# afermg/aliby

Hardware: AMD Instinct MI355X
Metric: FOV tiles/sec (whole node) (higher is better)
Workload: dtype u16 pixels, f64 feature accumulators, f32 dynamics, bfloat16 U-Net

## Files before the change

aliby_amd/csrc/feat_coloc.hip:

```cpp
#include "common.h"
#include "object_launch.h"
#include "coloc_stats.h"

typedef unsigned short u16;

struct ColocArgs {
  const u16* labels;
  const void* planes;
  int F, C, Y, X, ch0, ch1;
  const aliby_object* tab;
  int n_obj;
  int cap;
  unsigned char* gscratch;
  double* out;
  int ld;
  int col_pearson, col_manders, col_rwc, col_costes;
  double thr;
  double scale_max;
  const unsigned int* ranks;
  const int* rmax;
};

struct PlaneRanks {
  const unsigned int* rk1;
  const unsigned int* rk2;
  const int* rmax;
  int ch0, ch1;
  __device__ __forceinline__ double R() const { return (double)(max(rmax[ch0], rmax[ch1]) + 1); }
  __device__ __forceinline__ long long diff(int j) const { return llabs((long long)rk1[j] - (long long)rk2[j]); }
};

template <typename T, bool GLOBAL>
__global__ __launch_bounds__(256) void k_coloc(ColocArgs a) {
  extern __shared__ __align__(16) unsigned char lds_raw[];
  __shared__ double vec[4 * 8];
  __shared__ double red_d[8];
  __shared__ float red_f[8];
  __shared__ int red_i[8];
  __shared__ int wsum[4];
  unsigned char* ws = GLOBAL ? (a.gscratch + (size_t)blockIdx.x * (size_t)a.cap * 16) : lds_raw;
  float* fv = reinterpret_cast<float*>(ws);
  float* sv = fv + a.cap;
  unsigned int* rk1 = reinterpret_cast<unsigned int*>(sv + a.cap);
  unsigned int* rk2 = rk1 + a.cap;
  const int tid = threadIdx.x;
  const size_t plane = (size_t)a.Y * a.X;

  for (int oi = blockIdx.x; oi < a.n_obj; oi += gridDim.x) {
    const aliby_object o = a.tab[oi];
    double* out = a.out + (size_t)oi * a.ld;
    if (o.area <= 0) {
      if (tid == 0) {
        if (a.col_pearson >= 0) { out[a.col_pearson] = NAN; out[a.col_pearson + 1] = NAN; }
        if (a.col_manders >= 0) { out[a.col_manders] = NAN; out[a.col_manders + 1] = NAN; }
        if (a.col_rwc >= 0) { out[a.col_rwc] = NAN; out[a.col_rwc + 1] = NAN; }
        if (a.col_costes >= 0) { out[a.col_costes] = NAN; out[a.col_costes + 1] = NAN; }
      }
      continue;
    }
    const u16* lab = a.labels + (size_t)o.tile * plane;
    const T* p0 = reinterpret_cast<const T*>(a.planes) + ((size_t)o.tile * a.C + a.ch0) * plane;
    const T* p1 = reinterpret_cast<const T*>(a.planes) + ((size_t)o.tile * a.C + a.ch1) * plane;
    const int h = o.y1 - o.y0, w = o.x1 - o.x0, npix = h * w;
    const u16 L = (u16)o.label;

    __syncthreads();
    int base = 0;
    for (int i0 = 0; i0 < npix; i0 += blockDim.x) {
      const int i = i0 + tid;
      bool in = false;
      size_t idx = 0;
      if (i < npix) {
        idx = (size_t)(o.y0 + i / w) * a.X + (o.x0 + i % w);
        in = lab[idx] == L;
      }
      const int pos = block_compact_slot(in, base, wsum);
      if (in) {
        fv[pos] = px_load<T>(p0, idx); sv[pos] = px_load<T>(p1, idx);
        if (a.col_rwc >= 0) {
          rk1[pos] = a.ranks[((size_t)o.tile * a.C + a.ch0) * plane + idx];
          rk2[pos] = a.ranks[((size_t)o.tile * a.C + a.ch1) * plane + idx];
        }
      }
    }
    __syncthreads();
    const int N = base;
    coloc_block_stats(fv, sv, N, out, a.col_pearson, a.col_manders, a.col_rwc, a.col_costes, a.thr, a.scale_max,
                      PlaneRanks{rk1, rk2, a.rmax + (size_t)oi * a.C, a.ch0, a.ch1}, vec, red_f, red_i);
    (void)red_d;
    __syncthreads();
  }
}


#define COLOC_MAX_CH 8
#define COLOC_MAX_PAIRS 28
struct PairsArgs {
  const u16* labels;
  const void* planes;
  int F, C, Y, X;
  const aliby_object* tab;
  int n_obj, cap;
  double* out;
  int ld;
  double thr, scale_max;
  const unsigned int* ranks;
  const int* rmax;
  int nch, npairs, any_rwc;
  int chan[COLOC_MAX_CH];
  int pair[COLOC_MAX_PAIRS][6];
};

template <int K>
__device__ __forceinline__ void wave_sum_all(double (&v)[K]) {
#pragma unroll
  for (int k = 0; k < K; ++k) v[k] = wave_sum(v[k]);
}

template <typename T>
__global__ __launch_bounds__(256) void k_coloc_pairs(PairsArgs a) {
  extern __shared__ __align__(16) unsigned char lds_raw[];
  __shared__ int wsum[4];
  float* vals = reinterpret_cast<float*>(lds_raw);
  unsigned int* rks = reinterpret_cast<unsigned int*>(vals + (size_t)a.nch * a.cap);
  const int tid = threadIdx.x, lane = tid & 63, wave = tid >> 6;
  const size_t plane = (size_t)a.Y * a.X;

  for (int oi = blockIdx.x; oi < a.n_obj; oi += gridDim.x) {
    const aliby_object o = a.tab[oi];
    double* out = a.out + (size_t)oi * a.ld;
    if (o.area <= 0) {
      for (int p = tid; p < a.npairs; p += blockDim.x)
        for (int k = 2; k < 6; ++k)
          if (a.pair[p][k] >= 0) { out[a.pair[p][k]] = NAN; out[a.pair[p][k] + 1] = NAN; }
      continue;
    }
    const u16* lab = a.labels + (size_t)o.tile * plane;
    const T* img = reinterpret_cast<const T*>(a.planes) + (size_t)o.tile * a.C * plane;
    const int h = o.y1 - o.y0, w = o.x1 - o.x0, npix = h * w;
    const u16 L = (u16)o.label;
    __syncthreads();
    int base = 0;
    for (int i0 = 0; i0 < npix; i0 += blockDim.x) {
      const int i = i0 + tid;
      bool in = false;
      size_t idx = 0;
      if (i < npix) {
        idx = (size_t)(o.y0 + i / w) * a.X + (o.x0 + i % w);
        in = lab[idx] == L;
      }
      const int pos = block_compact_slot(in, base, wsum);
      if (in) {
        for (int c = 0; c < a.nch; ++c) {
          vals[(size_t)c * a.cap + pos] = px_load<T>(img + (size_t)a.chan[c] * plane, idx);
          if (a.any_rwc) rks[(size_t)c * a.cap + pos] = a.ranks[((size_t)o.tile * a.C + a.chan[c]) * plane + idx];
        }
      }
    }
    __syncthreads();
    const int N = base;
    const double dN = (double)N;

    for (int p = wave; p < a.npairs; p += 4) {
      const int ca = a.pair[p][0], cb = a.pair[p][1];
      const int col_pearson = a.pair[p][2], col_manders = a.pair[p][3], col_rwc = a.pair[p][4], col_costes = a.pair[p][5];
      const float* fv = vals + (size_t)ca * a.cap;
      const float* sv = vals + (size_t)cb * a.cap;
      const unsigned int* rk1 = rks + (size_t)ca * a.cap;
      const unsigned int* rk2 = rks + (size_t)cb * a.cap;

      double s2[2] = {0, 0};
      float m1 = -INFINITY, m2 = -INFINITY;
      for (int j = lane; j < N; j += 64) {
        s2[0] += (double)fv[j]; s2[1] += (double)sv[j];
        m1 = fmaxf(m1, fv[j]); m2 = fmaxf(m2, sv[j]);
      }
      wave_sum_all<2>(s2);
      const double mean1 = s2[0] / dN, mean2 = s2[1] / dN;
      const float MAX1 = wave_max(m1), MAX2 = wave_max(m2);

      if (col_pearson >= 0) {
        double q[3] = {0, 0, 0};
        for (int j = lane; j < N; j += 64) {
          const double x = (double)fv[j] - mean1, y = (double)sv[j] - mean2;
          q[0] += x * x; q[1] += y * y; q[2] += x * y;
        }
        wave_sum_all<3>(q);
        if (lane == 0) {
          out[col_pearson] = q[2] / (sqrt(q[0]) * sqrt(q[1]));
          out[col_pearson + 1] = q[2] / q[0];
        }
      }

      const double tff = (a.thr / 100.0) * (double)MAX1, tss = (a.thr / 100.0) * (double)MAX2;
      double tot1 = 0, tot2 = 0;
      int any_comb = 0;
      if (col_manders >= 0 || col_rwc >= 0) {
        double q[4] = {0, 0, 0, 0};
        int anyc = 0;
        for (int j = lane; j < N; j += 64) {
          const double f = fv[j], s = sv[j];
          const bool a1 = f >= tff, a2 = s >= tss;
          if (a1) q[0] += f;
          if (a2) q[1] += s;
          if (a1 && a2) { q[2] += f; q[3] += s; anyc = 1; }
        }
        wave_sum_all<4>(q);
        any_comb = wave_max(anyc);
        tot1 = q[0]; tot2 = q[1];
        if (col_manders >= 0 && lane == 0) {
          out[col_manders] = any_comb ? q[2] / tot1 : 0.0;
          out[col_manders + 1] = any_comb ? q[3] / tot2 : 0.0;
        }
      }

      if (col_rwc >= 0) {
        const double R = (double)(max(a.rmax[(size_t)oi * a.C + a.chan[ca]], a.rmax[(size_t)oi * a.C + a.chan[cb]]) + 1);
        double q[2] = {0, 0};
        for (int j = lane; j < N; j += 64) {
          const double f = fv[j], s = sv[j];
          if (f >= tff && s >= tss) {
            const long long di = llabs((long long)rk1[j] - (long long)rk2[j]);
            const double wgt = (R - (double)di) * 1.0 / R;
            q[0] += f * wgt; q[1] += s * wgt;
          }
        }
        wave_sum_all<2>(q);
        if (lane == 0) {
          out[col_rwc] = any_comb ? q[0] / tot1 : 0.0;
          out[col_rwc + 1] = any_comb ? q[1] / tot2 : 0.0;
        }
      }

      if (col_costes >= 0) {
        double q[3] = {0, 0, 0};
        for (int j = lane; j < N; j += 64) {
          const double f = fv[j], s = sv[j];
          if (f > 0 || s > 0) { q[0] += 1; q[1] += f; q[2] += s; }
        }
        wave_sum_all<3>(q);
        const double nnz = q[0], xmean = q[1] / nnz, ymean = q[2] / nnz, zmean = (q[1] + q[2]) / nnz;
        double v3[3] = {0, 0, 0};
        for (int j = lane; j < N; j += 64) {
          const double f = fv[j], s = sv[j];
          if (f > 0 || s > 0) {
            const double dx = f - xmean, dy = s - ymean, dz = (f + s) - zmean;
            v3[0] += dx * dx; v3[1] += dy * dy; v3[2] += dz * dz;
          }
        }
        wave_sum_all<3>(v3);
        const double xvar = v3[0] / (nnz - 1), yvar = v3[1] / (nnz - 1), zvar = v3[2] / (nnz - 1);
        const double covar = 0.5 * (zvar - (xvar + yvar));
        const double denom = 2 * covar;
        const double num = (yvar - xvar) + sqrt((yvar - xvar) * (yvar - xvar) + 4 * (covar * covar));
        const double cA = num / denom, cB = ymean - cA * xmean;
        double left = 1, right = a.scale_max;
      const bool int_bounds = a.scale_max == floor(a.scale_max) && a.scale_max >= 1 && a.scale_max <= 1048576.0;
        double mid = floor((right - left) / (6.0 / 5.0)) + left;
        double lastmid = 0, valid = 1;
        for (int it = 0; it < 200 && lastmid != mid; ++it) {
          const double t1 = mid / a.scale_max, t2 = cA * t1 + cB;
          double c3[3] = {0, 0, 0};
          for (int j = lane; j < N; j += 64) {
            const double f = fv[j], s = sv[j];
            if (f < t1 || s < t2) { c3[0] += 1; c3[1] += f; c3[2] += s; }
          }
          wave_sum_all<3>(c3);
          if (c3[0] <= 2) {
            left = mid - 1;
          } else {
            const double mx = c3[1] / c3[0], my = c3[2] / c3[0];
            double p3[3] = {0, 0, 0};
            for (int j = lane; j < N; j += 64) {
              const double f = fv[j], s = sv[j];
              if (f < t1 || s < t2) { const double dx = f - mx, dy = s - my; p3[0] += dx * dx; p3[1] += dy * dy; p3[2] += dx * dy; }
            }
            wave_sum_all<3>(p3);
            if (p3[0] != 0 && p3[1] != 0) {
              if (p3[2] < 0) left = mid - 1;
              else if (p3[2] >= 0) { right = mid + 1; valid = mid; }
            }
          }
          lastmid = mid;
          mid = costes_next_mid(left, right, int_bounds);
        }
        const double t1 = (valid - 1) / a.scale_max, t2 = cA * t1 + cB;
        double c4[4] = {0, 0, 0, 0};
        int f_any = 0, s_any = 0, c_any = 0;
        for (int j = lane; j < N; j += 64) {
          const double f = fv[j], s = sv[j];
          const bool fa = f > t1, sa = s > t2;
          f_any |= fa; s_any |= sa;
          if (f >= t1) c4[0] += f;
          if (s >= t2) c4[1] += s;
          if (fa && sa) { c4[2] += f; c4[3] += s; c_any = 1; }
        }
        wave_sum_all<4>(c4);
        const int FA = wave_max(f_any), SA = wave_max(s_any), CA = wave_max(c_any);
        if (lane == 0) {
          const double d1 = FA ? c4[0] : 0.0, d2 = SA ? c4[1] : 0.0;
          out[col_costes] = CA ? c4[2] / d1 : 0.0;
          out[col_costes + 1] = CA ? c4[3] / d2 : 0.0;
        }
      }
    }
  }
}


struct RankArgs {
  const u16* labels;
  const void* planes;
  int F, C, Y, X, channel;
  const aliby_object* tab;
  int n_obj, cap;
  unsigned char* gscratch;
  unsigned int* ranks;
  int* rmax;
};

template <typename T, bool GLOBAL>
__global__ __launch_bounds__(256) void k_ranks(RankArgs a) {
  extern __shared__ __align__(16) unsigned char lds_raw[];
  __shared__ int wsum[4];
  __shared__ int part[256];
  unsigned char* ws = GLOBAL ? (a.gscratch + (size_t)blockIdx.x * (size_t)a.cap * 16) : lds_raw;
  float* vals = reinterpret_cast<float*>(ws);
  float* S = vals + a.cap;
  int* P = reinterpret_cast<int*>(S + a.cap);
  int* pix = P + a.cap;
  const int tid = threadIdx.x;
  const size_t plane = (size_t)a.Y * a.X;
  for (int oi = blockIdx.x; oi < a.n_obj; oi += gridDim.x) {
    const aliby_object o = a.tab[oi];
    if (o.area <= 0) { if (tid == 0) a.rmax[(size_t)oi * a.C + a.channel] = 0; continue; }
    const u16* lab = a.labels + (size_t)o.tile * plane;
    const T* px = reinterpret_cast<const T*>(a.planes) + ((size_t)o.tile * a.C + a.channel) * plane;
    unsigned int* rk = a.ranks + ((size_t)o.tile * a.C + a.channel) * plane;
    const int h = o.y1 - o.y0, w = o.x1 - o.x0, npix = h * w;
    const u16 L = (u16)o.label;
    __syncthreads();
    int base = 0;
    for (int i0 = 0; i0 < npix; i0 += blockDim.x) {
      const int i = i0 + tid;
      bool in = false;
      size_t idx = 0;
      if (i < npix) { idx = (size_t)(o.y0 + i / w) * a.X + (o.x0 + i % w); in = lab[idx] == L; }
      const int pos = block_compact_slot(in, base, wsum);
      if (in) { vals[pos] = px_load<T>(px, idx); pix[pos] = (int)idx; }
    }
    __syncthreads();
    const int N = base;
    bool done = false;
    if (sizeof(T) == 2 && !GLOBAL) {
      int lo = INT_MAX, hi = 0;
      for (int j = tid; j < N; j += blockDim.x) { const int v = (int)vals[j]; lo = min(lo, v); hi = max(hi, v); }
      const int vmin = block_min_i32(lo, part), vmax = block_max_i32(hi, part);
      const int w0 = vmin >> 5, nw = (vmax >> 5) - w0 + 1;
      if (nw <= a.cap) {
        unsigned int* bits = reinterpret_cast<unsigned int*>(S);
        __syncthreads();
        for (int i = tid; i < nw; i += blockDim.x) bits[i] = 0u;
        __syncthreads();
        for (int j = tid; j < N; j += blockDim.x) { const int v = (int)vals[j]; atomicOr(&bits[(v >> 5) - w0], 1u << (v & 31)); }
        __syncthreads();
        for (int i = tid; i < nw; i += blockDim.x) P[i] = __popc(bits[i]);
        __syncthreads();
        block_inclusive_scan(P, nw, part);
        for (int j = tid; j < N; j += blockDim.x) {
          const int v = (int)vals[j], wi = (v >> 5) - w0;
          const unsigned int below = bits[wi] & ((1u << (v & 31)) - 1u);
          rk[pix[j]] = (unsigned int)(P[wi] - __popc(bits[wi]) + __popc(below));
        }
        if (tid == 0) a.rmax[(size_t)oi * a.C + a.channel] = P[nw - 1] - 1;
        done = true;
      }
    }
    if (done) { __syncthreads(); continue; }
    const int n2 = next_pow2(N);
    for (int i = tid; i < n2; i += blockDim.x) S[i] = (i < N) ? vals[i] : INFINITY;
    block_bitonic_sort(S, n2);
    for (int i = tid; i < N; i += blockDim.x) P[i] = (i > 0 && S[i] != S[i - 1]) ? 1 : 0;
    __syncthreads();
    block_inclusive_scan(P, N, part);
    for (int j = tid; j < N; j += blockDim.x) {
      const float v = vals[j];
      int lo = 0, hi = N;
      while (lo < hi) { const int mid = (lo + hi) >> 1; if (S[mid] < v) lo = mid + 1; else hi = mid; }
      rk[pix[j]] = (unsigned int)P[lo];
    }
    if (tid == 0) a.rmax[(size_t)oi * a.C + a.channel] = P[N - 1];
    __syncthreads();
  }
}

extern "C" int aliby_object_ranks(aliby_ctx* ctx, const uint16_t* labels, const void* planes, int dtype, int F, int C,
                                  int Y, int X, int channel, const aliby_object* table_dev, int n_obj, int max_area,
                                  uint32_t* ranks_dev, int32_t* rmax_dev, void* stream) {
  ARG_CHECK(ctx != nullptr, "ctx is NULL");
  if (n_obj == 0) return ALIBY_OK;
  ARG_CHECK(labels && planes && table_dev && ranks_dev && rmax_dev, "NULL argument");
  ARG_CHECK(dtype == ALIBY_U16 || dtype == ALIBY_F32, "dtype must be ALIBY_U16 or ALIBY_F32");
  ARG_CHECK(channel >= 0 && channel < C, "channel out of range");
  ARG_CHECK((size_t)Y * X < (size_t)INT_MAX, "plane too large");
  RankArgs a;
  a.labels = labels; a.planes = planes; a.F = F; a.C = C; a.Y = Y; a.X = X; a.channel = channel; a.tab = table_dev;
  a.n_obj = n_obj; a.ranks = ranks_dev; a.rmax = rmax_dev;
  a.cap = aliby_pow2_at_least(max_area, 64);
  return object_launch(ctx, object_kernel(dtype, k_ranks<u16, false>, k_ranks<float, false>),
                       object_kernel(dtype, k_ranks<u16, true>, k_ranks<float, true>), a, n_obj, (size_t)a.cap * 16, 96 * 1024, max_area,
                       as_stream(stream));
}

extern "C" int aliby_features_coloc(aliby_ctx* ctx, const uint16_t* labels, const void* planes, int dtype,
                                    int F, int C, int Y, int X, int ch0, int ch1,
                                    const aliby_object* table_dev, int n_obj, int max_area,
                                    double* out, int ld, int col_pearson, int col_manders, int col_rwc,
                                    int col_costes, double thr_percent, double costes_scale_max,
                                    const uint32_t* ranks_dev, const int32_t* rmax_dev, void* stream) {
  ARG_CHECK(ctx != nullptr, "ctx is NULL");
  if (n_obj == 0) return ALIBY_OK;
  ARG_CHECK(labels && planes && table_dev && out, "NULL argument");
  ARG_CHECK(dtype == ALIBY_U16 || dtype == ALIBY_F32, "dtype must be ALIBY_U16 or ALIBY_F32");
  ARG_CHECK(ch0 >= 0 && ch0 < C && ch1 >= 0 && ch1 < C, "channel out of range");
  ARG_CHECK(F > 0 && Y > 0 && X > 0 && max_area >= 0, "bad shape");
  const int cols[4] = {col_pearson, col_manders, col_rwc, col_costes};
  for (int k = 0; k < 4; ++k) ARG_CHECK(cols[k] < 0 || cols[k] + 2 <= ld, "columns exceed row stride");
  ColocArgs a;
  a.labels = labels; a.planes = planes; a.F = F; a.C = C; a.Y = Y; a.X = X; a.ch0 = ch0; a.ch1 = ch1;
  a.tab = table_dev; a.n_obj = n_obj; a.out = out; a.ld = ld;
  a.col_pearson = col_pearson; a.col_manders = col_manders; a.col_rwc = col_rwc; a.col_costes = col_costes;
  a.thr = thr_percent; a.scale_max = costes_scale_max;
  a.ranks = ranks_dev; a.rmax = rmax_dev;
  ARG_CHECK(col_rwc < 0 || (ranks_dev && rmax_dev), "rwc needs the rank planes (aliby_object_ranks)");
  a.cap = aliby_pow2_at_least(max_area, 64);
  return object_launch(ctx, object_kernel(dtype, k_coloc<u16, false>, k_coloc<float, false>),
                       object_kernel(dtype, k_coloc<u16, true>, k_coloc<float, true>), a, n_obj, (size_t)a.cap * 16, 96 * 1024, max_area,
                       as_stream(stream));
}

extern "C" int aliby_features_coloc_pairs(aliby_ctx* ctx, const uint16_t* labels, const void* planes, int dtype, int F, int C,
                                          int Y, int X, const int32_t* pairs_host, int n_pairs,
                                          const aliby_object* table_dev, int n_obj, int max_area, double* out, int ld,
                                          double thr_percent, double costes_scale_max, const uint32_t* ranks_dev,
                                          const int32_t* rmax_dev, void* stream) {
  ARG_CHECK(ctx != nullptr, "ctx is NULL");
  if (n_obj == 0 || n_pairs == 0) return ALIBY_OK;
  ARG_CHECK(labels && planes && table_dev && out && pairs_host, "NULL argument");
  ARG_CHECK(dtype == ALIBY_U16 || dtype == ALIBY_F32, "dtype must be ALIBY_U16 or ALIBY_F32");
  ARG_CHECK(F > 0 && Y > 0 && X > 0 && max_area >= 0, "bad shape");
  ARG_CHECK(n_pairs > 0 && n_pairs <= COLOC_MAX_PAIRS, "too many channel pairs for one launch");
  PairsArgs a;
  a.labels = labels; a.planes = planes; a.F = F; a.C = C; a.Y = Y; a.X = X; a.tab = table_dev; a.n_obj = n_obj;
  a.out = out; a.ld = ld; a.thr = thr_percent; a.scale_max = costes_scale_max; a.ranks = ranks_dev; a.rmax = rmax_dev;
  a.nch = 0; a.npairs = n_pairs; a.any_rwc = 0;
  for (int p = 0; p < n_pairs; ++p) {
    const int32_t* q = pairs_host + 6 * p;
    for (int k = 0; k < 2; ++k) {
      ARG_CHECK(q[k] >= 0 && q[k] < C, "channel out of range");
      int loc = -1;
      for (int c = 0; c < a.nch; ++c) if (a.chan[c] == q[k]) loc = c;
      if (loc < 0) {
        ARG_CHECK(a.nch < COLOC_MAX_CH, "too many distinct channels for one launch");
        loc = a.nch;
        a.chan[a.nch++] = q[k];
      }
      a.pair[p][k] = loc;
    }
    for (int k = 2; k < 6; ++k) {
      ARG_CHECK(q[k] < 0 || q[k] + 2 <= ld, "columns exceed row stride");
      a.pair[p][k] = q[k];
    }
    if (q[4] >= 0) a.any_rwc = 1;
  }
  ARG_CHECK(!a.any_rwc || (ranks_dev && rmax_dev), "rwc needs the rank planes (aliby_object_ranks)");
  a.cap = aliby_pow2_at_least(max_area, 64);
  const size_t need = (size_t)a.nch * a.cap * 4 * (a.any_rwc ? 2 : 1);
  if (need > 144 * 1024) {
    aliby_set_error("coloc_pairs: %zu bytes of pixel lists per object exceed the LDS budget", need);
    return ALIBY_ERR_TOO_LARGE;
  }
  hipStream_t s = as_stream(stream);
  auto k = object_kernel(dtype, k_coloc_pairs<u16>, k_coloc_pairs<float>);
  HIP_TRY(hipFuncSetAttribute((const void*)k, hipFuncAttributeMaxDynamicSharedMemorySize, 144 * 1024));
  hipLaunchKernelGGL(k, dim3(n_obj), dim3(256), need, s, a);
  KERNEL_CHECK();
  return ALIBY_OK;
}
```

Measured before the change: 604.4.

## Shrink LDS pixel and rank lists to u16 and window the rank bitset

The coloc pairs kernel now stores u16 pixel values and u16 ranks in LDS instead of float/uint32, sizes lists to a multiple of 64 rather than a power of two, and skips the shared-memory attribute call when it is not needed. For u16 inputs, the rank kernel gets a dedicated path that keeps u16 values and 16-bit positions in LDS. It builds the dense-rank bitset in fixed 256-word windows in static LDS, so the sort fallback is no longer used. The aim is to cut LDS footprint so more blocks fit per CU, and to avoid the bitonic sort. The cost is extra per-window passes when the value range is wide, plus a rescan path for very large objects.

```diff
diff --git a/aliby_amd/csrc/feat_coloc.hip b/aliby_amd/csrc/feat_coloc.hip
--- a/aliby_amd/csrc/feat_coloc.hip
+++ b/aliby_amd/csrc/feat_coloc.hip
@@ -95,6 +95,7 @@
 
 #define COLOC_MAX_CH 8
 #define COLOC_MAX_PAIRS 28
+#define COLOC_PAIRS_LDS_BUDGET (144 * 1024)
 struct PairsArgs {
   const u16* labels;
   const void* planes;
@@ -117,12 +118,24 @@
   for (int k = 0; k < K; ++k) v[k] = wave_sum(v[k]);
 }
 
+template <typename T> struct PairRank { typedef unsigned int type; };
+template <> struct PairRank<u16> { typedef u16 type; };
+static_assert((1u << (8 * sizeof(u16))) - 1u <= (PairRank<u16>::type)~0u, "the largest dense rank of uint16 pixels must fit the rank lists");
+
+static inline int list_cap64(int max_area) { return max_area <= 64 ? 64 : (max_area + 63) / 64 * 64; }
+static inline size_t coloc_pairs_need(int dtype, int nch, int cap, int any_rwc) {
+  const size_t v = dtype == ALIBY_U16 ? sizeof(u16) : sizeof(float);
+  const size_t r = dtype == ALIBY_U16 ? sizeof(PairRank<u16>::type) : sizeof(PairRank<float>::type);
+  return (size_t)nch * cap * (v + (any_rwc ? r : 0));
+}
+
 template <typename T>
 __global__ __launch_bounds__(256) void k_coloc_pairs(PairsArgs a) {
+  typedef typename PairRank<T>::type R;
   extern __shared__ __align__(16) unsigned char lds_raw[];
   __shared__ int wsum[4];
-  float* vals = reinterpret_cast<float*>(lds_raw);
-  unsigned int* rks = reinterpret_cast<unsigned int*>(vals + (size_t)a.nch * a.cap);
+  T* vals = reinterpret_cast<T*>(lds_raw);
+  R* rks = reinterpret_cast<R*>(vals + (size_t)a.nch * a.cap);
   const int tid = threadIdx.x, lane = tid & 63, wave = tid >> 6;
   const size_t plane = (size_t)a.Y * a.X;
 
@@ -152,8 +165,8 @@
       const int pos = block_compact_slot(in, base, wsum);
       if (in) {
         for (int c = 0; c < a.nch; ++c) {
-          vals[(size_t)c * a.cap + pos] = px_load<T>(img + (size_t)a.chan[c] * plane, idx);
-          if (a.any_rwc) rks[(size_t)c * a.cap + pos] = a.ranks[((size_t)o.tile * a.C + a.chan[c]) * plane + idx];
+          vals[(size_t)c * a.cap + pos] = img[(size_t)a.chan[c] * plane + idx];
+          if (a.any_rwc) rks[(size_t)c * a.cap + pos] = (R)a.ranks[((size_t)o.tile * a.C + a.chan[c]) * plane + idx];
         }
       }
     }
@@ -164,16 +177,16 @@
     for (int p = wave; p < a.npairs; p += 4) {
       const int ca = a.pair[p][0], cb = a.pair[p][1];
       const int col_pearson = a.pair[p][2], col_manders = a.pair[p][3], col_rwc = a.pair[p][4], col_costes = a.pair[p][5];
-      const float* fv = vals + (size_t)ca * a.cap;
-      const float* sv = vals + (size_t)cb * a.cap;
-      const unsigned int* rk1 = rks + (size_t)ca * a.cap;
-      const unsigned int* rk2 = rks + (size_t)cb * a.cap;
+      const T* fv = vals + (size_t)ca * a.cap;
+      const T* sv = vals + (size_t)cb * a.cap;
+      const R* rk1 = rks + (size_t)ca * a.cap;
+      const R* rk2 = rks + (size_t)cb * a.cap;
 
       double s2[2] = {0, 0};
       float m1 = -INFINITY, m2 = -INFINITY;
       for (int j = lane; j < N; j += 64) {
-        s2[0] += (double)fv[j]; s2[1] += (double)sv[j];
-        m1 = fmaxf(m1, fv[j]); m2 = fmaxf(m2, sv[j]);
+        s2[0] += (double)(float)fv[j]; s2[1] += (double)(float)sv[j];
+        m1 = fmaxf(m1, (float)fv[j]); m2 = fmaxf(m2, (float)sv[j]);
       }
       wave_sum_all<2>(s2);
       const double mean1 = s2[0] / dN, mean2 = s2[1] / dN;
@@ -182,7 +195,7 @@
       if (col_pearson >= 0) {
         double q[3] = {0, 0, 0};
         for (int j = lane; j < N; j += 64) {
-          const double x = (double)fv[j] - mean1, y = (double)sv[j] - mean2;
+          const double x = (double)(float)fv[j] - mean1, y = (double)(float)sv[j] - mean2;
           q[0] += x * x; q[1] += y * y; q[2] += x * y;
         }
         wave_sum_all<3>(q);
@@ -199,7 +212,7 @@
         double q[4] = {0, 0, 0, 0};
         int anyc = 0;
         for (int j = lane; j < N; j += 64) {
-          const double f = fv[j], s = sv[j];
+          const double f = (float)fv[j], s = (float)sv[j];
           const bool a1 = f >= tff, a2 = s >= tss;
           if (a1) q[0] += f;
           if (a2) q[1] += s;
@@ -218,7 +231,7 @@
         const double R = (double)(max(a.rmax[(size_t)oi * a.C + a.chan[ca]], a.rmax[(size_t)oi * a.C + a.chan[cb]]) + 1);
         double q[2] = {0, 0};
         for (int j = lane; j < N; j += 64) {
-          const double f = fv[j], s = sv[j];
+          const double f = (float)fv[j], s = (float)sv[j];
           if (f >= tff && s >= tss) {
             const long long di = llabs((long long)rk1[j] - (long long)rk2[j]);
             const double wgt = (R - (double)di) * 1.0 / R;
@@ -235,14 +248,14 @@
       if (col_costes >= 0) {
         double q[3] = {0, 0, 0};
         for (int j = lane; j < N; j += 64) {
-          const double f = fv[j], s = sv[j];
+          const double f = (float)fv[j], s = (float)sv[j];
           if (f > 0 || s > 0) { q[0] += 1; q[1] += f; q[2] += s; }
         }
         wave_sum_all<3>(q);
         const double nnz = q[0], xmean = q[1] / nnz, ymean = q[2] / nnz, zmean = (q[1] + q[2]) / nnz;
         double v3[3] = {0, 0, 0};
         for (int j = lane; j < N; j += 64) {
-          const double f = fv[j], s = sv[j];
+          const double f = (float)fv[j], s = (float)sv[j];
           if (f > 0 || s > 0) {
             const double dx = f - xmean, dy = s - ymean, dz = (f + s) - zmean;
             v3[0] += dx * dx; v3[1] += dy * dy; v3[2] += dz * dz;
@@ -262,7 +275,7 @@
           const double t1 = mid / a.scale_max, t2 = cA * t1 + cB;
           double c3[3] = {0, 0, 0};
           for (int j = lane; j < N; j += 64) {
-            const double f = fv[j], s = sv[j];
+            const double f = (float)fv[j], s = (float)sv[j];
             if (f < t1 || s < t2) { c3[0] += 1; c3[1] += f; c3[2] += s; }
           }
           wave_sum_all<3>(c3);
@@ -272,7 +285,7 @@
             const double mx = c3[1] / c3[0], my = c3[2] / c3[0];
             double p3[3] = {0, 0, 0};
             for (int j = lane; j < N; j += 64) {
-              const double f = fv[j], s = sv[j];
+              const double f = (float)fv[j], s = (float)sv[j];
               if (f < t1 || s < t2) { const double dx = f - mx, dy = s - my; p3[0] += dx * dx; p3[1] += dy * dy; p3[2] += dx * dy; }
             }
             wave_sum_all<3>(p3);
@@ -288,7 +301,7 @@
         double c4[4] = {0, 0, 0, 0};
         int f_any = 0, s_any = 0, c_any = 0;
         for (int j = lane; j < N; j += 64) {
-          const double f = fv[j], s = sv[j];
+          const double f = (float)fv[j], s = (float)sv[j];
           const bool fa = f > t1, sa = s > t2;
           f_any |= fa; s_any |= sa;
           if (f >= t1) c4[0] += f;
@@ -319,78 +332,122 @@
   int* rmax;
 };
 
+#define RANK_WINDOW_WORDS 256
+
 template <typename T, bool GLOBAL>
 __global__ __launch_bounds__(256) void k_ranks(RankArgs a) {
   extern __shared__ __align__(16) unsigned char lds_raw[];
   __shared__ int wsum[4];
   __shared__ int part[256];
-  unsigned char* ws = GLOBAL ? (a.gscratch + (size_t)blockIdx.x * (size_t)a.cap * 16) : lds_raw;
-  float* vals = reinterpret_cast<float*>(ws);
-  float* S = vals + a.cap;
-  int* P = reinterpret_cast<int*>(S + a.cap);
-  int* pix = P + a.cap;
   const int tid = threadIdx.x;
   const size_t plane = (size_t)a.Y * a.X;
-  for (int oi = blockIdx.x; oi < a.n_obj; oi += gridDim.x) {
-    const aliby_object o = a.tab[oi];
-    if (o.area <= 0) { if (tid == 0) a.rmax[(size_t)oi * a.C + a.channel] = 0; continue; }
-    const u16* lab = a.labels + (size_t)o.tile * plane;
-    const T* px = reinterpret_cast<const T*>(a.planes) + ((size_t)o.tile * a.C + a.channel) * plane;
-    unsigned int* rk = a.ranks + ((size_t)o.tile * a.C + a.channel) * plane;
-    const int h = o.y1 - o.y0, w = o.x1 - o.x0, npix = h * w;
-    const u16 L = (u16)o.label;
-    __syncthreads();
-    int base = 0;
-    for (int i0 = 0; i0 < npix; i0 += blockDim.x) {
-      const int i = i0 + tid;
-      bool in = false;
-      size_t idx = 0;
-      if (i < npix) { idx = (size_t)(o.y0 + i / w) * a.X + (o.x0 + i % w); in = lab[idx] == L; }
-      const int pos = block_compact_slot(in, base, wsum);
-      if (in) { vals[pos] = px_load<T>(px, idx); pix[pos] = (int)idx; }
-    }
-    __syncthreads();
-    const int N = base;
-    bool done = false;
-    if (sizeof(T) == 2 && !GLOBAL) {
+  if constexpr (sizeof(T) == 2 && !GLOBAL) {
+    __shared__ unsigned int bits[RANK_WINDOW_WORDS];
+    __shared__ int P[RANK_WINDOW_WORDS];
+    u16* vals = reinterpret_cast<u16*>(lds_raw);
+    u16* pos = vals + a.cap;
+    for (int oi = blockIdx.x; oi < a.n_obj; oi += gridDim.x) {
+      const aliby_object o = a.tab[oi];
+      if (o.area <= 0) { if (tid == 0) a.rmax[(size_t)oi * a.C + a.channel] = 0; continue; }
+      const u16* lab = a.labels + (size_t)o.tile * plane;
+      const T* px = reinterpret_cast<const T*>(a.planes) + ((size_t)o.tile * a.C + a.channel) * plane;
+      unsigned int* rk = a.ranks + ((size_t)o.tile * a.C + a.channel) * plane;
+      const int h = o.y1 - o.y0, w = o.x1 - o.x0, npix = h * w;
+      const u16 L = (u16)o.label;
+      const bool pos16 = npix <= 65536;
+      __syncthreads();
+      int base = 0;
+      for (int i0 = 0; i0 < npix; i0 += blockDim.x) {
+        const int i = i0 + tid;
+        bool in = false;
+        size_t idx = 0;
+        if (i < npix) { idx = (size_t)(o.y0 + i / w) * a.X + (o.x0 + i % w); in = lab[idx] == L; }
+        const int slot = block_compact_slot(in, base, wsum);
+        if (in) { vals[slot] = px[idx]; if (pos16) pos[slot] = (u16)i; }
+      }
+      __syncthreads();
+      const int N = base;
       int lo = INT_MAX, hi = 0;
-      for (int j = tid; j < N; j += blockDim.x) { const int v = (int)vals[j]; lo = min(lo, v); hi = max(hi, v); }
+      for (int j = tid; j < N; j += blockDim.x) { const int v = vals[j]; lo = min(lo, v); hi = max(hi, v); }
       const int vmin = block_min_i32(lo, part), vmax = block_max_i32(hi, part);
-      const int w0 = vmin >> 5, nw = (vmax >> 5) - w0 + 1;
-      if (nw <= a.cap) {
-        unsigned int* bits = reinterpret_cast<unsigned int*>(S);
+      const int w0 = vmin >> 5, nw = N > 0 ? (vmax >> 5) - w0 + 1 : 0;
+      int below_window = 0;
+      for (int wb = 0; wb < nw; wb += RANK_WINDOW_WORDS) {
+        const int wlo = w0 + wb, n = min(nw - wb, RANK_WINDOW_WORDS);
         __syncthreads();
-        for (int i = tid; i < nw; i += blockDim.x) bits[i] = 0u;
+        for (int i = tid; i < n; i += blockDim.x) bits[i] = 0u;
         __syncthreads();
-        for (int j = tid; j < N; j += blockDim.x) { const int v = (int)vals[j]; atomicOr(&bits[(v >> 5) - w0], 1u << (v & 31)); }
+        for (int j = tid; j < N; j += blockDim.x) {
+          const int v = vals[j], wi = (v >> 5) - wlo;
+          if ((unsigned int)wi < (unsigned int)n) atomicOr(&bits[wi], 1u << (v & 31));
+        }
         __syncthreads();
-        for (int i = tid; i < nw; i += blockDim.x) P[i] = __popc(bits[i]);
+        for (int i = tid; i < n; i += blockDim.x) P[i] = __popc(bits[i]);
         __syncthreads();
-        block_inclusive_scan(P, nw, part);
-        for (int j = tid; j < N; j += blockDim.x) {
-          const int v = (int)vals[j], wi = (v >> 5) - w0;
-          const unsigned int below = bits[wi] & ((1u << (v & 31)) - 1u);
-          rk[pix[j]] = (unsigned int)(P[wi] - __popc(bits[wi]) + __popc(below));
-        }
-        if (tid == 0) a.rmax[(size_t)oi * a.C + a.channel] = P[nw - 1] - 1;
-        done = true;
-      }
-    }
-    if (done) { __syncthreads(); continue; }
-    const int n2 = next_pow2(N);
-    for (int i = tid; i < n2; i += blockDim.x) S[i] = (i < N) ? vals[i] : INFINITY;
-    block_bitonic_sort(S, n2);
-    for (int i = tid; i < N; i += blockDim.x) P[i] = (i > 0 && S[i] != S[i - 1]) ? 1 : 0;
-    __syncthreads();
-    block_inclusive_scan(P, N, part);
-    for (int j = tid; j < N; j += blockDim.x) {
-      const float v = vals[j];
-      int lo = 0, hi = N;
-      while (lo < hi) { const int mid = (lo + hi) >> 1; if (S[mid] < v) lo = mid + 1; else hi = mid; }
-      rk[pix[j]] = (unsigned int)P[lo];
-    }
-    if (tid == 0) a.rmax[(size_t)oi * a.C + a.channel] = P[N - 1];
-    __syncthreads();
+        block_inclusive_scan(P, n, part);
+        if (pos16) {
+          for (int j = tid; j < N; j += blockDim.x) {
+            const int v = vals[j], wi = (v >> 5) - wlo;
+            if ((unsigned int)wi >= (unsigned int)n) continue;
+            const int i = pos[j];
+            const unsigned int below = bits[wi] & ((1u << (v & 31)) - 1u);
+            rk[(size_t)(o.y0 + i / w) * a.X + (o.x0 + i % w)] = (unsigned int)(below_window + P[wi] - __popc(bits[wi]) + __popc(below));
+          }
+        } else {
+          for (int i = tid; i < npix; i += blockDim.x) {
+            const size_t idx = (size_t)(o.y0 + i / w) * a.X + (o.x0 + i % w);
+            if (lab[idx] != L) continue;
+            const int v = px[idx], wi = (v >> 5) - wlo;
+            if ((unsigned int)wi >= (unsigned int)n) continue;
+            const unsigned int below = bits[wi] & ((1u << (v & 31)) - 1u);
+            rk[idx] = (unsigned int)(below_window + P[wi] - __popc(bits[wi]) + __popc(below));
+          }
+        }
+        below_window += P[n - 1];
+      }
+      if (tid == 0) a.rmax[(size_t)oi * a.C + a.channel] = below_window - 1;
+    }
+  } else {
+    unsigned char* ws = GLOBAL ? (a.gscratch + (size_t)blockIdx.x * (size_t)a.cap * 16) : lds_raw;
+    float* vals = reinterpret_cast<float*>(ws);
+    float* S = vals + a.cap;
+    int* P = reinterpret_cast<int*>(S + a.cap);
+    int* pix = P + a.cap;
+    for (int oi = blockIdx.x; oi < a.n_obj; oi += gridDim.x) {
+      const aliby_object o = a.tab[oi];
+      if (o.area <= 0) { if (tid == 0) a.rmax[(size_t)oi * a.C + a.channel] = 0; continue; }
+      const u16* lab = a.labels + (size_t)o.tile * plane;
+      const T* px = reinterpret_cast<const T*>(a.planes) + ((size_t)o.tile * a.C + a.channel) * plane;
+      unsigned int* rk = a.ranks + ((size_t)o.tile * a.C + a.channel) * plane;
+      const int h = o.y1 - o.y0, w = o.x1 - o.x0, npix = h * w;
+      const u16 L = (u16)o.label;
+      __syncthreads();
+      int base = 0;
+      for (int i0 = 0; i0 < npix; i0 += blockDim.x) {
+        const int i = i0 + tid;
+        bool in = false;
+        size_t idx = 0;
+        if (i < npix) { idx = (size_t)(o.y0 + i / w) * a.X + (o.x0 + i % w); in = lab[idx] == L; }
+        const int pos = block_compact_slot(in, base, wsum);
+        if (in) { vals[pos] = px_load<T>(px, idx); pix[pos] = (int)idx; }
+      }
+      __syncthreads();
+      const int N = base;
+      const int n2 = next_pow2(N);
+      for (int i = tid; i < n2; i += blockDim.x) S[i] = (i < N) ? vals[i] : INFINITY;
+      block_bitonic_sort(S, n2);
+      for (int i = tid; i < N; i += blockDim.x) P[i] = (i > 0 && S[i] != S[i - 1]) ? 1 : 0;
+      __syncthreads();
+      block_inclusive_scan(P, N, part);
+      for (int j = tid; j < N; j += blockDim.x) {
+        const float v = vals[j];
+        int lo = 0, hi = N;
+        while (lo < hi) { const int mid = (lo + hi) >> 1; if (S[mid] < v) lo = mid + 1; else hi = mid; }
+        rk[pix[j]] = (unsigned int)P[lo];
+      }
+      if (tid == 0) a.rmax[(size_t)oi * a.C + a.channel] = P[N - 1];
+      __syncthreads();
+    }
   }
 }
 
@@ -407,8 +464,13 @@
   a.labels = labels; a.planes = planes; a.F = F; a.C = C; a.Y = Y; a.X = X; a.channel = channel; a.tab = table_dev;
   a.n_obj = n_obj; a.ranks = ranks_dev; a.rmax = rmax_dev;
   a.cap = aliby_pow2_at_least(max_area, 64);
+  const size_t need = (size_t)a.cap * 16, budget = 96 * 1024;
+  if (dtype == ALIBY_U16 && need <= budget) {
+    a.cap = list_cap64(max_area);
+    return object_launch(ctx, k_ranks<u16, false>, k_ranks<u16, true>, a, n_obj, (size_t)a.cap * 4, budget, max_area, as_stream(stream));
+  }
   return object_launch(ctx, object_kernel(dtype, k_ranks<u16, false>, k_ranks<float, false>),
-                       object_kernel(dtype, k_ranks<u16, true>, k_ranks<float, true>), a, n_obj, (size_t)a.cap * 16, 96 * 1024, max_area,
+                       object_kernel(dtype, k_ranks<u16, true>, k_ranks<float, true>), a, n_obj, need, budget, max_area,
                        as_stream(stream));
 }
 
@@ -474,15 +536,16 @@
     if (q[4] >= 0) a.any_rwc = 1;
   }
   ARG_CHECK(!a.any_rwc || (ranks_dev && rmax_dev), "rwc needs the rank planes (aliby_object_ranks)");
-  a.cap = aliby_pow2_at_least(max_area, 64);
-  const size_t need = (size_t)a.nch * a.cap * 4 * (a.any_rwc ? 2 : 1);
-  if (need > 144 * 1024) {
-    aliby_set_error("coloc_pairs: %zu bytes of pixel lists per object exceed the LDS budget", need);
+  const size_t routed = (size_t)a.nch * aliby_pow2_at_least(max_area, 64) * 4 * (a.any_rwc ? 2 : 1);
+  if (routed > COLOC_PAIRS_LDS_BUDGET) {
+    aliby_set_error("coloc_pairs: %zu bytes of pixel lists per object exceed the LDS budget", routed);
     return ALIBY_ERR_TOO_LARGE;
   }
+  a.cap = list_cap64(max_area);
+  const size_t need = coloc_pairs_need(dtype, a.nch, a.cap, a.any_rwc);
   hipStream_t s = as_stream(stream);
   auto k = object_kernel(dtype, k_coloc_pairs<u16>, k_coloc_pairs<float>);
-  HIP_TRY(hipFuncSetAttribute((const void*)k, hipFuncAttributeMaxDynamicSharedMemorySize, 144 * 1024));
+  if (need > OBJECT_LDS_ATTR_ABOVE) HIP_TRY(hipFuncSetAttribute((const void*)k, hipFuncAttributeMaxDynamicSharedMemorySize, COLOC_PAIRS_LDS_BUDGET));
   hipLaunchKernelGGL(k, dim3(n_obj), dim3(256), need, s, a);
   KERNEL_CHECK();
   return ALIBY_OK;
```

Result: no change. 607.3, median of 6 (+0.5%).
